# skywoodsz/qm_control

Measured on NVIDIA H100. Metric: mpc_wbc_iters_per_s, higher is better.
Workload: dtype f64

## Files before the change

### qm_control_b200/csrc/kernels/wbc_kernel.cu

```cuda
#include "dev_common.cuh"
#include "payload.cuh"
#include "wlinalg.cuh"

namespace qmb {

constexpr int LDM = 25;
constexpr int LDZ = 37;
constexpr int LZ = 19;
constexpr int MAXR = 24;
constexpr int LJC = 9;
constexpr int MAXW = 20;
#ifndef QMB_WBC_WARPS
#define QMB_WBC_WARPS 8
#endif
constexpr int WBC_WARPS = QMB_WBC_WARPS;

enum { ST_OK = 0, ST_ITER_CAP = 1, ST_TOO_MANY_ROWS = 2, ST_NAN = 4 };

struct EeWs { double Jee[6 * LDM], djv_ee[6], ee_m_pos[3], ee_m_vel[3], ee_m_rot[9], ee_m_w[3], ee_d_pos[3], ee_d_vel[3], ee_d_rot[9]; };
struct QpWs {
  union ZA { struct Q { double Z[36 * LZ];
                        double AR[MAXR * LDZ];
                      } q;
             RbdWs rbd;
             __device__ ZA() {} } za;
  union AH { double Ah[MAXR * LZ];
             EeWs ee; __device__ AH() {} } ah;
  double G[18 * 19 / 2 + 1];
  double tau[MAXR], tauc[MAXW];
  double xbar[36], dx[36], g[36], y[36], s[36], zac[LZ + 1], rhs[MAXR], bp[MAXR], bh[MAXR], lam[MAXW], t18[MAXR];
  int perm[MAXR], permc[MAXW], wset[MAXW];
};
static_assert(LZ * MAXR + LZ * MAXW <= MAXR * LDZ, "W1 and Wc share the row build area");
static_assert(sizeof(RbdWs) <= sizeof(double) * (36 * LZ + MAXR * LDZ), "rigid-body workspace overlays Z + AR only");

struct WbcSmem {
  double q[NQ], v[NQ], qd[NQ], vd[NQ];
  double M[NQ * LDM], nle[NQ];
  double Jc[12 * LJC], djv_f[12], fpos_m[12], fvel_m[12], fpos_d[12], fvel_d[12];
  double Tm[9], wdot_base[3], base_acc[6], fdes[12], lim[NJ], vstar[56];
  QpWs qp;
  Tuning tun;
};

struct IneqCtx { const WbcSmem* sm; int mode; int nc; double mu; int lfp, ffp; };
__device__ __forceinline__ int foot_first(int ffp, int f) { return (ffp >> (4 * f)) & 15; }
__device__ __forceinline__ double jt_force(const WbcSmem* sm, int lfp, int jn, const double* F) {
  if (jn >= 12) return 0.0;
  const int lg = jn / 3, f = (lfp >> (2 * lg)) & 3, d = jn - 3 * lg; const double* J = sm->Jc + 3 * f * LJC + 6 + d;
  return J[0] * F[3 * f] + J[LJC] * F[3 * f + 1] + J[2 * LJC] * F[3 * f + 2];
}

__device__ __forceinline__ int stance_foot_by_rank(int mode, int rank) { int k = 0; for (int f = 0; f < 4; ++f) if (contact_flag(mode, f)) { if (k == rank) return f; ++k; } return -1; }

__device__ __forceinline__ double ineq_row_dot(const IneqCtx& c, int i, const double* x) {
  if (i < 36) {
    const int jn = i < 18 ? i : i - 18; const double* Mr = c.sm->M + (6 + jn) * LDM; double s = 0.0;
    for (int k = 0; k < NQ; ++k) s += Mr[k] * x[k];
    s -= jt_force(c.sm, c.lfp, jn, x + NQ);
    return i < 18 ? s : -s;
  }
  const int r = i - 36; const int foot = stance_foot_by_rank(c.mode, r / 5); const int t = r % 5; const double* F = x + NQ + 3 * foot;
  if (t == 0) return -F[2];
  if (t == 1) return F[0] - c.mu * F[2];
  if (t == 2) return -F[0] - c.mu * F[2];
  if (t == 3) return F[1] - c.mu * F[2];
  return -F[1] - c.mu * F[2];
}
__device__ __forceinline__ double ineq_rhs(const IneqCtx& c, int i) {
  double f = 0.0;
  if (i < 18) f = c.sm->lim[i] - c.sm->nle[6 + i]; else if (i < 36) f = c.sm->lim[i - 18] + c.sm->nle[6 + i - 18];
  return f + c.sm->vstar[i];
}
__device__ __forceinline__ double ineq_row_elem(const IneqCtx& c, int i, int k) {
  if (i < 36) { const int jn = i < 18 ? i : i - 18; const double sgn = i < 18 ? 1.0 : -1.0; if (k < NQ) return sgn * c.sm->M[(6 + jn) * LDM + k];
    const int r = k - NQ, d = jn - foot_first(c.ffp, r / 3); return (d >= 0 && d < 3) ? -sgn * c.sm->Jc[r * LJC + 6 + d] : 0.0; }
  const int r = i - 36; const int foot = stance_foot_by_rank(c.mode, r / 5); const int t = r % 5; const int kk = k - NQ - 3 * foot;
  if (kk < 0 || kk > 2) return 0.0;
  if (kk == 2) return t == 0 ? -1.0 : -c.mu;
  if (kk == 0) return t == 1 ? 1.0 : (t == 2 ? -1.0 : 0.0);
  return t == 3 ? 1.0 : (t == 4 ? -1.0 : 0.0);
}

__device__ int cod_lstsq(QpWs& qp, double* W, int n, int r, int ldw, const double* rhs, double* y, double* G, int lane) {
  const int k = w_qrcp(W, n, r, ldw, qp.tau, qp.perm, 1e-11, lane);
  for (int i = lane; i < n; i += 32) y[i] = 0.0;
  __syncwarp();
  if (k == 0) return 0;
  if (k == r) {
    for (int c = 0; c < k; ++c) {
      double part = 0.0; if (lane < c) part = W[lane + c * ldw] * y[lane];
      const double s = warp_sum(part);
      if (lane == 0) y[c] = (rhs[qp.perm[c]] - s) / W[c + c * ldw];
      __syncwarp();
    }
  } else {
    { int a = 0, b = lane; while (b > a) { b -= a + 1; ++a; }
      while (a < k) { double s = 0.0; for (int c = a; c < r; ++c) s += W[a + c * ldw] * W[b + c * ldw]; G[tri(a) + b] = s;
        b += 32; while (b > a) { b -= a + 1; ++a; } } }
    if (lane < k) { double s = 0.0; for (int c = lane; c < r; ++c) s += W[lane + c * ldw] * rhs[qp.perm[c]]; qp.t18[lane] = s; }
    __syncwarp();
    w_cholesky(G, k, lane);
    w_chol_solve(G, k, qp.t18, lane);
    if (lane < k) y[lane] = qp.t18[lane];
    __syncwarp();
  }
  w_apply_q(W, n, k, ldw, qp.tau, y, lane);
  return k;
}

__device__ int build_level(WbcSmem& sm, const Tuning* __restrict__ tn, int level, int mode, int variant, bool init_phase, int ffp, int lane) {
  QpWs& qp = sm.qp; double* Ap = qp.za.q.AR; const EeWs& ee = qp.ah.ee; int nc = 0; for (int f = 0; f < 4; ++f) nc += contact_flag(mode, f);
  int rows = 0;
  if (level == 0) rows = 18;
  else if (level == 1) rows = (variant == 0) ? (init_phase ? 6 : 10 + 3 * (4 - nc)) : (6 + 3 * (4 - nc));
  else rows = (variant == 0) ? 14 : 12;
  for (int e = lane; e < rows * LDZ; e += 32) Ap[e] = 0.0;
  __syncwarp();
  if (level == 0) {
    for (int e = lane; e < 6 * 36; e += 32) { const int r = e / 36, k = e % 36; Ap[r * LDZ + k] = (k < NQ) ? sm.M[r * LDM + k] : -sm.Jc[(k - NQ) * LJC + r]; }
    if (lane < 6) qp.bp[lane] = -sm.nle[lane];
    int row = 6;
    for (int f = 0; f < 4; ++f) if (contact_flag(mode, f)) { if (lane < 27) { const int a = lane / 9, c = lane - 9 * a; Ap[(row + a) * LDZ + (c < 6 ? c : foot_first(ffp, f) + c)] = sm.Jc[(3 * f + a) * LJC + c]; } if (lane < 3) qp.bp[row + lane] = -sm.djv_f[3 * f + lane]; row += 3; }
    for (int f = 0; f < 4; ++f) if (!contact_flag(mode, f)) { if (lane < 3) { Ap[(row + lane) * LDZ + NQ + 3 * f + lane] = 1.0; qp.bp[row + lane] = 0.0; } row += 3; }
  } else if (level == 1) {
    int row = 0;
    if (variant == 0 && init_phase) {
      if (lane < 6) { const int k = NQ - 6 + lane; Ap[lane * LDZ + k] = 1.0; qp.bp[lane] = tn->arm_joint_kp[lane] * (sm.qd[k] - sm.q[k]) + tn->arm_joint_kd[lane] * (sm.vd[k] - sm.v[k]); }
      row = 6;
    } else {
      if (lane == 0) { Ap[2] = 1.0; qp.bp[0] = sm.base_acc[2] + tn->base_height_kp * (sm.qd[2] - sm.q[2]) + tn->base_height_kd * (sm.vd[2] - sm.v[2]); }
      if (lane < 3) {
        const int r = lane; for (int k = 0; k < 3; ++k) Ap[(1 + r) * LDZ + 3 + k] = sm.Tm[3 * r + k];
        double wM[3], wD[3]; matvec3(sm.Tm, sm.v + 3, wM); matvec3(sm.Tm, sm.vd + 3, wD);
        double Rm[9], Rr[9], err[3]; rot_zyx(sm.q[3], sm.q[4], sm.q[5], Rm); rot_zyx(sm.qd[3], sm.qd[4], sm.qd[5], Rr); rotation_error_world(Rr, Rm, err);
        double tdd[3], tde[3]; matvec3(sm.Tm, sm.base_acc + 3, tdd); euler_rate_map_dot_times(sm.q[3], sm.q[4], sm.vd + 3, tde);
        qp.bp[1 + r] = tdd[r] + tde[r] + tn->base_angular_kp * err[r] + tn->base_angular_kd * (wD[r] - wM[r]) - sm.wdot_base[r];
      }
      row = 4;
      if (variant == 0) {
        for (int e = lane; e < 6 * NQ; e += 32) { const int a = e / NQ, k = e % NQ; const bool zero = (a >= 3 && k >= 3 && k < 6); Ap[(row + a) * LDZ + k] = zero ? 0.0 : ee.Jee[a * LDM + k]; }
        if (lane < 3) qp.bp[row + lane] = tn->ee_linear_kp[lane] * (ee.ee_d_pos[lane] - ee.ee_m_pos[lane]) + tn->ee_linear_kd[lane] * (ee.ee_d_vel[lane] - ee.ee_m_vel[lane]) - ee.djv_ee[lane];
        if (lane == 3) { double err[3]; rotation_error_world(ee.ee_d_rot, ee.ee_m_rot, err);
          for (int a = 0; a < 3; ++a) qp.bp[row + 3 + a] = tn->ee_angular_kp[a] * err[a] - tn->ee_angular_kd[a] * ee.ee_m_w[a] - (ee.djv_ee[3 + a] - sm.wdot_base[a]); }
        row += 6;
      } else {
        if (lane < 2) { Ap[(row + lane) * LDZ + lane] = 1.0; qp.bp[row + lane] = sm.base_acc[lane] + tn->base_linear_kp * (sm.qd[lane] - sm.q[lane]) + tn->base_linear_kd * (sm.vd[lane] - sm.v[lane]); }
        row += 2;
      }
      for (int f = 0; f < 4; ++f) if (!contact_flag(mode, f)) {
        if (lane < 27) { const int a = lane / 9, c = lane - 9 * a; Ap[(row + a) * LDZ + (c < 6 ? c : foot_first(ffp, f) + c)] = 100.0 * sm.Jc[(3 * f + a) * LJC + c]; }
        if (lane < 3) { const int i = 3 * f + lane; qp.bp[row + lane] = 100.0 * (tn->kp_swing * (sm.fpos_d[i] - sm.fpos_m[i]) + tn->kd_swing * (sm.fvel_d[i] - sm.fvel_m[i]) - sm.djv_f[i]); }
        row += 3;
      }
    }
  } else {
    if (lane < 12) { Ap[lane * LDZ + NQ + lane] = 1.0; qp.bp[lane] = sm.fdes[lane]; }
    if (variant == 0 && lane < 2) { Ap[(12 + lane) * LDZ + lane] = 1.0; qp.bp[12 + lane] = sm.base_acc[lane] + tn->base_linear_kp * (sm.qd[lane] - sm.q[lane]) + tn->base_linear_kd * (sm.vd[lane] - sm.v[lane]); }
  }
  __syncwarp();
  return rows;
}

__device__ __forceinline__ void project_task(QpWs& qp, int rows, int off, int nz, int lane) {
  const double* Ap = qp.za.q.AR; const double* Z = qp.za.q.Z;
  for (int e = lane; e < rows * nz; e += 32) { const int i = e / nz, c = e - i * nz; const double* a = Ap + i * LDZ; double s0 = 0.0, s1 = 0.0;
#pragma unroll 6
    for (int k = 0; k < 36; k += 2) { s0 = fma(a[k], Z[k * LZ + off + c], s0); s1 = fma(a[k + 1], Z[(k + 1) * LZ + off + c], s1); }
    qp.ah.Ah[i * LZ + c] = s0 + s1; }
  if (lane < rows) { const double* a = Ap + lane * LDZ; double s = 0.0; for (int k = 0; k < 36; ++k) s = fma(a[k], qp.xbar[k], s); qp.bh[lane] = qp.bp[lane] - s; }
  __syncwarp();
}

__device__ int solve_level(WbcSmem& sm, const IneqCtx& ic, int rows, int off, int nzc, int& nw, int lane, int& iters_out, int iter_cap) {
  QpWs& qp = sm.qp; const int nz = nzc - off; const int nineq = 36 + 5 * ic.nc; int status = 0;
  if (nz <= 0) return 0;
  const double* Z = qp.za.q.Z; const double* Ah = qp.ah.Ah; double* W1 = qp.za.q.AR; double* Wc = qp.za.q.AR + LZ * MAXR;
  if (lane < LZ + 1) qp.zac[lane] = 0.0;
  __syncwarp();
  bool converged = false;
  for (int iter = 0; iter < iter_cap; ++iter) {
    iters_out = iter + 1;
    int kc = 0;
    if (nw > 0) {
      for (int k = 0; k < nw; ++k) {
        const int wi = qp.wset[k]; qp.y[lane] = ineq_row_elem(ic, wi, lane); if (lane < 4) qp.y[32 + lane] = ineq_row_elem(ic, wi, 32 + lane);
        __syncwarp();
        if (lane < nz) { double s0 = 0.0, s1 = 0.0;
#pragma unroll 6
          for (int j = 0; j < 36; j += 2) { s0 = fma(qp.y[j], Z[j * LZ + off + lane], s0); s1 = fma(qp.y[j + 1], Z[(j + 1) * LZ + off + lane], s1); }
          Wc[lane + k * LZ] = s0 + s1; }
        __syncwarp();
      }
      kc = w_qrcp(Wc, nz, nw, LZ, qp.tauc, qp.permc, 1e-10, lane);
      if (kc < nw) {
        int keep = (lane < kc) ? qp.wset[qp.permc[lane]] : -1; __syncwarp(); if (lane < kc) qp.wset[lane] = keep; nw = kc; __syncwarp();
        continue;
      }
    }
    for (int e = lane; e < rows * LZ; e += 32) W1[e] = Ah[e];
    if (lane < rows) { const double* a = Ah + lane * LZ; double s = 0.0; for (int c = 0; c < nz; ++c) s = fma(a[c], qp.zac[c], s); qp.rhs[lane] = qp.bh[lane] - s; }
    __syncwarp();
    if (kc > 0) w_apply_qt_cols(Wc, nz, kc, LZ, qp.tauc, W1, rows, LZ, lane);
    const int nfree = nz - kc;
    for (int i = lane; i < nz; i += 32) qp.s[i] = 0.0;
    __syncwarp();
    if (nfree > 0) cod_lstsq(qp, W1 + kc, nfree, rows, LZ, qp.rhs, qp.s + kc, qp.G, lane);
    if (kc > 0) w_apply_q(Wc, nz, kc, LZ, qp.tauc, qp.s, lane);
    for (int i = lane; i < 36; i += 32) { double d = 0.0; for (int c = 0; c < nz; ++c) d = fma(Z[i * LZ + off + c], qp.s[c], d); qp.dx[i] = d; }
    __syncwarp();
    double dmax = 0.0, xmax = 0.0; for (int i = lane; i < 36; i += 32) { dmax = fmax(dmax, fabs(qp.dx[i])); xmax = fmax(xmax, fabs(qp.xbar[i])); }
    dmax = warp_max(dmax); xmax = warp_max(xmax);
    bool full_step = true;
    if (dmax > 1e-12 * (1.0 + xmax)) {
      double alpha = 1.0; int blk = -1;
      for (int i = lane; i < nineq; i += 32) {
        bool inw = false; for (int k = 0; k < nw; ++k) inw |= (qp.wset[k] == i);
        if (inw) continue;
        const double ad = ineq_row_dot(ic, i, qp.dx);
        if (ad > 1e-12 * (1.0 + dmax)) { double r = (ineq_rhs(ic, i) - ineq_row_dot(ic, i, qp.xbar)) / ad; if (r < 0.0) r = 0.0; if (r < alpha) { alpha = r; blk = i; } }
      }
      { double a = alpha; int b = (blk < 0) ? 0x7fffffff : blk; warp_argmin(a, b); alpha = a; blk = (alpha < 1.0) ? b : -1; }
      for (int i = lane; i < 36; i += 32) qp.xbar[i] += alpha * qp.dx[i];
      if (lane < nz) qp.zac[lane] += alpha * qp.s[lane];
      __syncwarp();
      if (blk >= 0) { if (nw >= MAXW) { status |= ST_TOO_MANY_ROWS; break; } if (lane == 0) qp.wset[nw] = blk; nw += 1; __syncwarp(); full_step = false; }
    }
    if (!full_step) continue;
    if (nw == 0) { converged = true; break; }
    if (lane < rows) { const double* a = Ah + lane * LZ; double s = 0.0; for (int c = 0; c < nz; ++c) s = fma(a[c], qp.zac[c], s); qp.rhs[lane] = s - qp.bh[lane]; }
    __syncwarp();
    for (int c = lane; c < nz; c += 32) { double s = 0.0; for (int r = 0; r < rows; ++r) s = fma(Ah[r * LZ + c], qp.rhs[r], s); qp.g[c] = s; }
    __syncwarp();
    w_apply_qt(Wc, nz, kc, LZ, qp.tauc, qp.g, lane);
    double gmax = 0.0; for (int i = lane; i < nz; i += 32) gmax = fmax(gmax, fabs(qp.g[i])); gmax = warp_max(gmax);
    for (int c = kc - 1; c >= 0; --c) {
      double part = 0.0; if (lane > c && lane < kc) part = Wc[c + lane * LZ] * qp.lam[lane];
      const double s = warp_sum(part);
      if (lane == 0) qp.lam[c] = (-qp.g[c] - s) / Wc[c + c * LZ];
      __syncwarp();
    }
    double lmin = (lane < kc) ? qp.lam[lane] : 1e300; int li = lane; warp_argmin(lmin, li);
    if (lmin >= -1e-9 * (1.0 + gmax)) { converged = true; break; }
    { const int drop = qp.permc[li]; int keep = -1; if (lane < nw) { int src = lane < drop ? lane : lane + 1; keep = (src < nw) ? qp.wset[src] : -1; } __syncwarp(); if (lane < nw - 1) qp.wset[lane] = keep;
      nw -= 1; __syncwarp(); }
  }
  if (!converged) status |= ST_ITER_CAP;
  return status;
}

template <bool TUNED>
__global__ void __launch_bounds__(32 * WBC_WARPS) wbc_update_kernel(const DevModel* __restrict__ mdl, int b0, int B, const double* __restrict__ x_des, const double* __restrict__ u_des,
                                                                   const double* __restrict__ rbd_meas, const int32_t* __restrict__ mode_in, const double* __restrict__ period_in,
                                                                   const double* __restrict__ time_in, double* __restrict__ input_last, int variant,
                                                                   double* __restrict__ cmd_out, int32_t* __restrict__ status_out, int32_t* __restrict__ diag_out,
                                                                   const double* __restrict__ srbd, const double* __restrict__ payload, const double* __restrict__ tuning) {
  extern __shared__ __align__(16) unsigned char smem_raw[];
  const int warp = threadIdx.x >> 5, lane = threadIdx.x & 31;
  const int b = b0 + blockIdx.x * (int)(blockDim.x >> 5) + warp;
  if (b >= B) return;
  WbcSmem& sm = reinterpret_cast<WbcSmem*>(smem_raw)[warp];
  const int mode = mode_in[b]; const double period = period_in[b]; const double time = time_in[b];
  int nc = 0; for (int f = 0; f < 4; ++f) nc += contact_flag(mode, f);

  const double* xdes = x_des + (size_t)b * NX; const double* udes = u_des + (size_t)b * NU;
  if (lane < 12) sm.fdes[lane] = udes[lane];
  const int lfp = mdl->leg_foot[0] | (mdl->leg_foot[1] << 2) | (mdl->leg_foot[2] << 4) | (mdl->leg_foot[3] << 6);
  const int ffp = mdl->foot_leg[0] | (mdl->foot_leg[1] << 4) | (mdl->foot_leg[2] << 8) | (mdl->foot_leg[3] << 12);
  if (lane < NJ) sm.lim[lane] = (lane < 12) ? mdl->effort[lane % 3] : mdl->effort[lane];
  for (int i = lane; i < 56; i += 32) sm.vstar[i] = 0.0;
  rbd_read(rbd_meas + (size_t)b * 55, sm.q, sm.v, sm.Tm, lane);
  if (lane < NQ) sm.qd[lane] = xdes[6 + lane];
  __syncwarp();

  RbdWs* ws = &sm.qp.za.rbd; EeWs& ee = sm.qp.ah.ee;
  rbd_kinematics<true>(mdl, sm.q, sm.v, ws, lane);
  rbd_inertias(mdl, ws, lane, 1);
  if (payload) { if (lane < 2) payload_load(mdl, ws, lane, payload + (size_t)b * 8 + 4 * lane, true); __syncwarp(); }
  rbd_accumulate(mdl, ws, lane, true);
  rbd_mass_matrix_nle(mdl, ws, sm.M, LDM, sm.nle, lane);
  for (int f = 0; f < 4; ++f) {
    const int body = mdl->foot_body[f]; double pw[3]; foot_point(mdl, ws, f, pw);
    if (lane < 9) { const double* S = ws->S[lane < 6 ? lane : foot_first(ffp, f) + lane]; double col[3]; point_vel(S, pw, col);
      for (int a = 0; a < 3; ++a) sm.Jc[(3 * f + a) * LJC + lane] = col[a]; }
    if (lane == 0) { double vel[3], acc[3]; point_vel_acc(ws->V[body], ws->A[body], pw, vel, acc); for (int a = 0; a < 3; ++a) { sm.fpos_m[3 * f + a] = pw[a]; sm.fvel_m[3 * f + a] = vel[a]; sm.djv_f[3 * f + a] = acc[a]; } }
  }
  {
    const int body = mdl->ee_body; double pw[3]; ee_pose(mdl, ws, pw, lane == 0 ? ee.ee_m_rot : nullptr);
    point_jacobian(ws, pw, 12, 17, ee.Jee, LDM, lane);
    if (lane < NQ) { const bool on = (lane < 6) || (lane >= 18); for (int a = 0; a < 3; ++a) ee.Jee[(3 + a) * LDM + lane] = on ? ws->S[lane][a] : 0.0; }
    if (lane == 0) { double vel[3], acc[3]; point_vel_acc(ws->V[body], ws->A[body], pw, vel, acc); for (int a = 0; a < 3; ++a) { ee.ee_m_pos[a] = pw[a]; ee.ee_m_vel[a] = vel[a]; ee.djv_ee[a] = acc[a]; ee.djv_ee[3 + a] = ws->A[body][a]; ee.ee_m_w[a] = ws->V[body][a]; sm.wdot_base[a] = ws->A[0][a]; } }
  }
  __syncwarp();

  double jacc = 0.0;
  if (lane < NJ) { const double uj = udes[12 + lane]; jacc = (uj - input_last[(size_t)b * NU + 12 + lane]) / period; sm.vd[6 + lane] = uj; }
  __syncwarp();
  if (lane < NU) input_last[(size_t)b * NU + lane] = udes[lane];
  double A22inv[9], A12[9];
  if (lane == 0) {
    const SrbdConst* sc = srbd_of(mdl, srbd, b);
    double R[9], T[9]; rot_zyx(sm.qd[3], sm.qd[4], sm.qd[5], R); euler_rate_map(sm.qd[3], sm.qd[4], T);
    double c[3]; matvec3(R, sc->c_nom, c);
    double RI[9], RIRt[9], A22[9]; matmul3(R, sc->I_nom, RI); matmul3_nt(RI, R, RIRt); matmul3(RIRt, T, A22); inv3(A22, A22inv);
    const double Sx[9] = {0, -c[2], c[1], c[2], 0, -c[0], -c[1], c[0], 0}; double ST[9]; matmul3(Sx, T, ST); for (int i = 0; i < 9; ++i) A12[i] = sc->m * ST[i];
    double ha[3] = {sc->m * xdes[3], sc->m * xdes[4], sc->m * xdes[5]}, ed[3]; matvec3(A22inv, ha, ed);
    double t[3]; matvec3(A12, ed, t);
    for (int a = 0; a < 3; ++a) { sm.vd[a] = xdes[a] - t[a] / sc->m; sm.vd[3 + a] = ed[a]; }
  }
  __syncwarp();
  rbd_kinematics<true>(mdl, sm.qd, sm.vd, ws, lane);
  rbd_inertias(mdl, ws, lane, 2);
  if (payload) { if (lane < 2) payload_load(mdl, ws, lane, payload + (size_t)b * 8 + 4 * lane, false); __syncwarp(); }
  rbd_accumulate(mdl, ws, lane, true);
  double Phi[6] = {0, 0, 0, 0, 0, 0};
  if (lane < NJ) { inertia_apply(ws->Ic[lane + 1], ws->S[6 + lane], Phi); for (int i = 0; i < 6; ++i) Phi[i] *= jacc; }
  for (int i = 0; i < 6; ++i) Phi[i] = warp_sum(Phi[i]);
  for (int f = 0; f < 4; ++f) {
    double pw[3]; foot_point(mdl, ws, f, pw);
    if (lane == 0) { double vel[3]; point_vel(ws->V[mdl->foot_body[f]], pw, vel); for (int a = 0; a < 3; ++a) { sm.fpos_d[3 * f + a] = pw[a]; sm.fvel_d[3 * f + a] = vel[a]; } }
  }
  if (lane == 0) {
    double pw[3], vel[3]; ee_pose(mdl, ws, pw, ee.ee_d_rot); point_vel(ws->V[mdl->ee_body], pw, vel);
    for (int a = 0; a < 3; ++a) { ee.ee_d_pos[a] = pw[a]; ee.ee_d_vel[a] = vel[a]; }
    const SrbdConst* sc = srbd_of(mdl, srbd, b);
    const double mt = ws->Ic[0][0]; const double com[3] = {ws->Ic[0][1] / mt, ws->Ic[0][2] / mt, ws->Ic[0][3] / mt};
    double lin[3] = {0, 0, -9.81 * sc->m}, ang[3] = {0, 0, 0};
    for (int f = 0; f < 4; ++f) { const double* F = sm.fdes + 3 * f; const double r[3] = {sm.fpos_d[3 * f] - com[0], sm.fpos_d[3 * f + 1] - com[1], sm.fpos_d[3 * f + 2] - com[2]}; lin[0] += F[0]; lin[1] += F[1]; lin[2] += F[2]; cross3_add(r, F, ang); }
    const double* Fb = ws->F[0]; double cf[3]; cross3(com, Fb + 3, cf);
    double cp[3]; cross3(com, Phi + 3, cp);
    for (int a = 0; a < 3; ++a) { lin[a] -= Fb[3 + a] + Phi[3 + a]; ang[a] -= (Fb[a] - cf[a]) + (Phi[a] - cp[a]); }
    double ed[3]; matvec3(A22inv, ang, ed); double t[3]; matvec3(A12, ed, t);
    for (int a = 0; a < 3; ++a) { sm.base_acc[a] = (lin[a] - t[a]) / sc->m; sm.base_acc[3 + a] = ed[a]; }
  }
  __syncwarp();

  if (TUNED) { const double* tr = tuning + (size_t)b * TUNING_DBL; for (int i = lane; i < TUNING_MODEL; i += 32) reinterpret_cast<double*>(&sm.tun)[i] = tr[i]; }
  const Tuning* tn = TUNED ? &sm.tun : tuning_of(mdl, nullptr, 0);
  QpWs& qp = sm.qp; IneqCtx ic{&sm, mode, nc, TUNED ? tuning[(size_t)b * TUNING_DBL + 1] : mdl->wbc_friction, lfp, ffp}; int status = 0;
  const bool init_phase = time < 10.0;
  double* AR = qp.za.q.AR; double* Z = qp.za.q.Z;
  for (int i = lane; i < 36; i += 32) qp.xbar[i] = 0.0;
  __syncwarp();
  const int nineq = 36 + 5 * nc; const int cap0 = mdl->wbc_iter_cap0, cap = mdl->wbc_iter_cap; int it0 = 0;
  unsigned vmask0 = 0, vmask1 = 0;
  int k0 = 0;
  for (int it = 0; it < cap0; ++it) {
    int r = build_level(sm, tn, 0, mode, variant, init_phase, ffp, lane); it0 = it + 1;
    for (int i = 0; i < nineq; ++i) { const bool in = (i < 32) ? ((vmask0 >> i) & 1u) : ((vmask1 >> (i - 32)) & 1u); if (in) { if (r >= MAXR) { status |= ST_TOO_MANY_ROWS; break; }
        for (int k = lane; k < 36; k += 32) AR[r * LDZ + k] = ineq_row_elem(ic, i, k); if (lane == 0) qp.bp[r] = ineq_rhs(ic, i); ++r; } }
    __syncwarp();
    k0 = cod_lstsq(qp, AR, 36, r, LDZ, qp.bp, qp.xbar, Z, lane);
    __syncwarp();
    unsigned n0 = 0, n1 = 0;
    for (int i = lane; i < nineq; i += 32) { const double val = ineq_row_dot(ic, i, qp.xbar) - ineq_rhs(ic, i); const double sc = 1e-9 * (1.0 + fabs(ineq_rhs(ic, i)));
      const bool inV = (i < 32) ? ((vmask0 >> i) & 1u) : ((vmask1 >> (i - 32)) & 1u);
      if (val > sc || (inV && val >= -sc)) { if (i < 32) n0 |= 1u << i; else n1 |= 1u << (i - 32); } }
    for (int o = 16; o > 0; o >>= 1) { n0 |= __shfl_xor_sync(FULL, n0, o); n1 |= __shfl_xor_sync(FULL, n1, o); }
    if (n0 == vmask0 && n1 == vmask1) break;
    vmask0 = n0; vmask1 = n1;
    if (it == cap0 - 1) status |= ST_ITER_CAP;
  }
  for (int i = lane; i < nineq; i += 32) { const double val = ineq_row_dot(ic, i, qp.xbar) - ineq_rhs(ic, i); sm.vstar[i] = val > 0.0 ? val : 0.0; }
  __syncwarp();
  int off = 0, nzc = 0, nw = 0, it1 = 0, it2 = 0;
  {
    if (vmask0 | vmask1) {
      const int rows0 = build_level(sm, tn, 0, mode, variant, init_phase, ffp, lane);
      k0 = w_qrcp(AR, 36, rows0, LDZ, qp.tau, qp.perm, 1e-11, lane);
    }
    nzc = 36 - k0;
    if (nzc > LZ - 1) { status |= ST_TOO_MANY_ROWS; nzc = 0; }
    else w_form_q_tail(AR, 36, k0, LDZ, qp.tau, Z, LZ, lane);
  }
  for (int level = 1; level <= 2 && nzc > 0; ++level) {
    const int rows = build_level(sm, tn, level, mode, variant, init_phase, ffp, lane);
    const int nz = nzc - off;
    if (nz <= 0) break;
    project_task(qp, rows, off, nz, lane);
    status |= solve_level(sm, ic, rows, off, nzc, nw, lane, level == 1 ? it1 : it2, cap);
    if (level == 1) {
      const int k = w_qrcp(qp.ah.Ah, nz, rows, LZ, qp.tau, qp.perm, 1e-11, lane);
      w_apply_q_right(qp.ah.Ah, nz, k, LZ, qp.tau, Z, 36, LZ, off, lane);
      off += k;
    }
  }
  double* out = cmd_out + (size_t)b * 54;
  for (int i = lane; i < 36; i += 32) out[i] = qp.xbar[i];
  bool bad = false;
  if (lane < NJ) { const double* Mr = sm.M + (6 + lane) * LDM; double s = sm.nle[6 + lane]; for (int k = 0; k < NQ; ++k) s += Mr[k] * qp.xbar[k]; s -= jt_force(&sm, lfp, lane, qp.xbar + NQ); out[36 + lane] = s; bad = !isfinite(s); }
  if (__any_sync(FULL, bad)) status |= ST_NAN;
  if (lane == 0) { status_out[b] = status; if (diag_out) diag_out[b] = (it0 & 0xff) | ((it1 & 0xff) << 8) | ((it2 & 0xff) << 16) | ((nw & 0xff) << 24); }
}

static_assert(sizeof(WbcSmem) * WBC_WARPS <= 227 * 1024, "WBC shared-memory budget exceeded");
size_t wbc_smem_bytes() { return sizeof(WbcSmem) * WBC_WARPS; }

void launch_wbc_update(const DevModel* mdl, int B, const double* x_des, const double* u_des, const double* rbd, const int32_t* mode, const double* period, const double* time,
                       double* input_last, int variant, double* cmd, int32_t* status, cudaStream_t stream, int b0, int b1, int32_t* diag, const double* srbd, const double* payload, const double* tuning) {
  if (b1 < 0) b1 = B; if (b1 <= b0) return;
  const int nb = b1 - b0; const int wpc = WBC_WARPS;
  const int grid = (nb + wpc - 1) / wpc;
  (tuning ? wbc_update_kernel<true> : wbc_update_kernel<false>)<<<grid, 32 * wpc, sizeof(WbcSmem) * wpc, stream>>>(mdl, b0, b1, x_des, u_des, rbd, mode, period, time, input_last, variant, cmd, status, diag, srbd, payload, tuning);
}

int wbc_configure_device() {
  cudaError_t e = cudaFuncSetAttribute(wbc_update_kernel<false>, cudaFuncAttributeMaxDynamicSharedMemorySize, (int)wbc_smem_bytes());
  if (e == cudaSuccess) e = cudaFuncSetAttribute(wbc_update_kernel<true>, cudaFuncAttributeMaxDynamicSharedMemorySize, (int)wbc_smem_bytes());
  return (int)e;
}

}
```

### qm_control_b200/csrc/kernels/wlinalg.cuh

```cuda
#pragma once
#include "dev_common.cuh"

#ifndef QMB_QRCP_NORMS
#define QMB_QRCP_NORMS 2
#endif

namespace qmb {


__device__ __forceinline__ int w_qrcp(double* W, int n, int r, int ld, double* tau, int* perm, double tol_rel, int lane) {
  if (lane < r) perm[lane] = lane;
  double vn = 0.0;
  if (lane < r) for (int i = 0; i < n; ++i) { const double x = W[i + lane * ld]; vn += x * x; }
  double vref = vn;
  const double thresh = tol_rel * tol_rel * warp_max(vn);
  const int kmax = n < r ? n : r; int rank = kmax;
  __syncwarp();
  for (int j = 0; j < kmax; ++j) {
#if QMB_QRCP_NORMS == 0
    if (lane >= j && lane < r) { vn = 0.0; for (int i = j; i < n; ++i) { const double x = W[i + lane * ld]; vn += x * x; } }
#endif
    double nr = vn; int pc = lane;
    warp_argmax_nonneg(nr, pc, lane >= j && lane < r);
    if (!(nr > thresh)) { rank = j; break; }
    if (pc != j) {
      for (int i = lane; i < n; i += 32) { const double t = W[i + j * ld]; W[i + j * ld] = W[i + pc * ld]; W[i + pc * ld] = t; }
      if (lane == 0) { const int t = perm[j]; perm[j] = perm[pc]; perm[pc] = t; }
      const double vj = __shfl_sync(FULL, vn, j), rj = __shfl_sync(FULL, vref, j);
      if (lane == pc) { vn = vj; vref = rj; }
    }
    __syncwarp();
#if QMB_QRCP_NORMS == 1
    {
      double part = 0.0; for (int i = j + lane; i < n; i += 32) { const double x = W[i + j * ld]; part += x * x; }
      nr = warp_sum(part);
      if (!(nr > thresh)) { rank = j; break; }
    }
#endif
    const double x0 = W[j + j * ld]; const double beta = (x0 >= 0.0) ? -sqrt(nr) : sqrt(nr);
    const double d = x0 - beta, inv = 1.0 / (beta * d);
    const double tj = -d * d * inv; const double scal = beta * inv;
    __syncwarp();
    for (int i = j + 1 + lane; i < n; i += 32) W[i + j * ld] *= scal;
    if (lane == 0) { W[j + j * ld] = beta; tau[j] = tj; }
    __syncwarp();
    if (lane > j && lane < r) {
      double* col = W + lane * ld; const double* v = W + j * ld;
      double w = col[j]; for (int i = j + 1; i < n; ++i) w += v[i] * col[i];
      w *= tj; const double cj = col[j] - w; col[j] = cj;
#if QMB_QRCP_NORMS == 2
      double nn = 0.0; for (int i = j + 1; i < n; ++i) { const double c = fma(-w, v[i], col[i]); col[i] = c; nn = fma(c, c, nn); }
      vn = nn;
#else
      for (int i = j + 1; i < n; ++i) col[i] -= w * v[i];
#endif
#if QMB_QRCP_NORMS == 1
      vn = fmax(vn - cj * cj, 0.0);
      if (vref > 0.0 && vn <= 1.4901161193847656e-8 * vref) {
        vn = 0.0; for (int i = j + 1; i < n; ++i) { const double x = col[i]; vn += x * x; }
        if (!(vn > thresh)) vn = 0.0;
        vref = vn;
      }
#endif
    }
    __syncwarp();
  }
  return rank;
}

__device__ __forceinline__ void w_apply_qt(const double* W, int n, int k, int ld, const double* tau, double* g, int lane) {
  for (int j = 0; j < k; ++j) {
    const double* v = W + j * ld; double part = 0.0;
    for (int i = j + lane; i < n; i += 32) part += (i == j ? 1.0 : v[i]) * g[i];
    const double w = tau[j] * warp_sum(part);
    for (int i = j + lane; i < n; i += 32) g[i] -= w * (i == j ? 1.0 : v[i]);
    __syncwarp();
  }
}
__device__ __forceinline__ void w_apply_q(const double* W, int n, int k, int ld, const double* tau, double* g, int lane) {
  for (int j = k - 1; j >= 0; --j) {
    const double* v = W + j * ld; double part = 0.0;
    for (int i = j + lane; i < n; i += 32) part += (i == j ? 1.0 : v[i]) * g[i];
    const double w = tau[j] * warp_sum(part);
    for (int i = j + lane; i < n; i += 32) g[i] -= w * (i == j ? 1.0 : v[i]);
    __syncwarp();
  }
}
__device__ __forceinline__ void w_apply_qt_cols(const double* W, int n, int k, int ld, const double* tau, double* C, int ncols, int ldc, int lane) {
  if (lane < ncols) {
    double* col = C + lane * ldc;
    for (int j = 0; j < k; ++j) {
      const double* v = W + j * ld; double w = col[j]; for (int i = j + 1; i < n; ++i) w = fma(v[i], col[i], w);
      w *= tau[j]; col[j] -= w; for (int i = j + 1; i < n; ++i) col[i] = fma(-w, v[i], col[i]);
    }
  }
  __syncwarp();
}
__device__ __forceinline__ void w_apply_q_right(const double* W, int n, int k, int ld, const double* tau, double* Z, int rows, int ldz, int off, int lane) {
  for (int j = 0; j < k; ++j) {
    const double* v = W + j * ld; const double tj = tau[j];
    for (int i = lane; i < rows; i += 32) {
      double* zr = Z + i * ldz + off; double d = zr[j]; for (int c = j + 1; c < n; ++c) d += zr[c] * v[c];
      d *= tj; zr[j] -= d; for (int c = j + 1; c < n; ++c) zr[c] -= d * v[c];
    }
    __syncwarp();
  }
}

__device__ __forceinline__ void w_form_q_tail(const double* W, int n, int k, int ld, const double* tau, double* Z, int ldz, int lane) {
  const int nc = n - k;
  if (lane < nc) {
    double* col = Z + lane;
    for (int i = 0; i < n; ++i) col[i * ldz] = (i == k + lane) ? 1.0 : 0.0;
    for (int j = k - 1; j >= 0; --j) {
      const double* v = W + j * ld; double w0 = col[j * ldz], w1 = 0.0; int i = j + 1;
      for (; i + 1 < n; i += 2) { w0 = fma(v[i], col[i * ldz], w0); w1 = fma(v[i + 1], col[(i + 1) * ldz], w1); }
      if (i < n) w0 = fma(v[i], col[i * ldz], w0);
      const double w = (w0 + w1) * tau[j]; col[j * ldz] -= w; for (int i2 = j + 1; i2 < n; ++i2) col[i2 * ldz] = fma(-w, v[i2], col[i2 * ldz]);
    }
  }
  __syncwarp();
}

__device__ __forceinline__ int tri(int a) { return (a * (a + 1)) >> 1; }
__device__ __forceinline__ bool w_cholesky(double* A, int n, int lane) {
  bool ok = true;
  for (int j = 0; j < n; ++j) {
    const double d = A[tri(j) + j];
    if (!(d > 0.0)) { ok = false; break; }
    const double s = sqrt(d);
    __syncwarp();
    double* row = A + tri(lane);
    if (lane == j) row[j] = s;
    if (lane > j && lane < n) row[j] /= s;
    __syncwarp();
    if (lane > j && lane < n) { const double lij = row[j]; int oc = tri(j + 1) + j; for (int c = j + 1; c <= lane; ++c) { row[c] -= lij * A[oc]; oc += c + 1; } }
    __syncwarp();
  }
  return ok;
}
__device__ __forceinline__ void w_chol_solve(const double* L, int n, double* b, int lane) {
  const double* row = L + tri(lane);
  for (int j = 0; j < n; ++j) {
    if (lane == j) b[j] /= row[j];
    __syncwarp();
    if (lane > j && lane < n) b[lane] -= row[j] * b[j];
    __syncwarp();
  }
  for (int j = n - 1; j >= 0; --j) {
    if (lane == j) b[j] /= row[j];
    __syncwarp();
    if (lane < j) b[lane] -= L[tri(j) + lane] * b[j];
    __syncwarp();
  }
}

}
```

Before: 24.37.

## Update working-set QR incrementally and reuse level-0 factorisation across passes

The active-set QP inner loop now keeps Ah and zac in the rotated basis and appends a newly blocking constraint to the existing Householder QR of the working set. Previously it re-projected every working constraint and reran a full pivoted QR on each iteration; a full refactorisation now happens only after a constraint is dropped or an append is rank-deficient. The level-0 factorisation from the first semismooth pass is cached in Z/bh and restored later instead of being rebuilt, and several dot-product loops are split into two or four accumulators. In exchange the numerics change slightly, there is extra rotate/unrotate bookkeeping, and the cached factorisation depends on aliasing shared workspace correctly.

```diff
diff --git a/qm_control_b200/csrc/kernels/wbc_kernel.cu b/qm_control_b200/csrc/kernels/wbc_kernel.cu
--- a/qm_control_b200/csrc/kernels/wbc_kernel.cu
+++ b/qm_control_b200/csrc/kernels/wbc_kernel.cu
@@ -32,6 +32,7 @@
   int perm[MAXR], permc[MAXW], wset[MAXW];
 };
 static_assert(LZ * MAXR + LZ * MAXW <= MAXR * LDZ, "W1 and Wc share the row build area");
+static_assert(18 * 36 <= 36 * LZ && 18 <= MAXR, "Z and bh hold the level-0 factorisation of A0 (18 rows) between the semismooth passes");
 static_assert(sizeof(RbdWs) <= sizeof(double) * (36 * LZ + MAXR * LDZ), "rigid-body workspace overlays Z + AR only");
 
 struct WbcSmem {
@@ -172,42 +173,68 @@
   __syncwarp();
 }
 
+__device__ __forceinline__ double project_ineq_row(QpWs& qp, const IneqCtx& ic, int i, int off, int nz, int lane) {
+  const double* Z = qp.za.q.Z;
+  qp.y[lane] = ineq_row_elem(ic, i, lane); if (lane < 4) qp.y[32 + lane] = ineq_row_elem(ic, i, 32 + lane);
+  __syncwarp();
+  double d = 0.0;
+  if (lane < nz) { double s0 = 0.0, s1 = 0.0, s2 = 0.0, s3 = 0.0;
+#pragma unroll 3
+    for (int j = 0; j < 36; j += 4) { s0 = fma(qp.y[j], Z[j * LZ + off + lane], s0); s1 = fma(qp.y[j + 1], Z[(j + 1) * LZ + off + lane], s1);
+                                      s2 = fma(qp.y[j + 2], Z[(j + 2) * LZ + off + lane], s2); s3 = fma(qp.y[j + 3], Z[(j + 3) * LZ + off + lane], s3); }
+    d = (s0 + s1) + (s2 + s3); }
+  __syncwarp();
+  return d;
+}
+
 __device__ int solve_level(WbcSmem& sm, const IneqCtx& ic, int rows, int off, int nzc, int& nw, int lane, int& iters_out, int iter_cap) {
   QpWs& qp = sm.qp; const int nz = nzc - off; const int nineq = 36 + 5 * ic.nc; int status = 0;
   if (nz <= 0) return 0;
-  const double* Z = qp.za.q.Z; const double* Ah = qp.ah.Ah; double* W1 = qp.za.q.AR; double* Wc = qp.za.q.AR + LZ * MAXR;
+  const double* Z = qp.za.q.Z; double* Ah = qp.ah.Ah; double* W1 = qp.za.q.AR; double* Wc = qp.za.q.AR + LZ * MAXR;
   if (lane < LZ + 1) qp.zac[lane] = 0.0;
   __syncwarp();
+  int kc = 0;
+  bool refactor = nw > 0;
+  double cmax = 0.0;
   bool converged = false;
   for (int iter = 0; iter < iter_cap; ++iter) {
     iters_out = iter + 1;
-    int kc = 0;
-    if (nw > 0) {
-      for (int k = 0; k < nw; ++k) {
-        const int wi = qp.wset[k]; qp.y[lane] = ineq_row_elem(ic, wi, lane); if (lane < 4) qp.y[32 + lane] = ineq_row_elem(ic, wi, 32 + lane);
-        __syncwarp();
-        if (lane < nz) { double s0 = 0.0, s1 = 0.0;
-#pragma unroll 6
-          for (int j = 0; j < 36; j += 2) { s0 = fma(qp.y[j], Z[j * LZ + off + lane], s0); s1 = fma(qp.y[j + 1], Z[(j + 1) * LZ + off + lane], s1); }
-          Wc[lane + k * LZ] = s0 + s1; }
-        __syncwarp();
-      }
+    if (!refactor && nw > kc) {
+      const double c = project_ineq_row(qp, ic, qp.wset[kc], off, nz, lane);
+      cmax = fmax(cmax, warp_sum(c * c));
+      if (w_qr_append(Wc, nz, kc, LZ, qp.tauc, c, 1e-20 * cmax, lane)) {
+        w_apply_qt_cols(Wc, nz, kc + 1, LZ, qp.tauc, Ah, rows, LZ, lane, kc); w_apply_qt(Wc, nz, kc + 1, LZ, qp.tauc, qp.zac, lane, kc);
+        kc += 1;
+      } else refactor = true;
+    }
+    if (refactor) {
+      refactor = false;
+      if (kc > 0) { w_apply_q_cols(Wc, nz, kc, LZ, qp.tauc, Ah, rows, LZ, lane); w_apply_q(Wc, nz, kc, LZ, qp.tauc, qp.zac, lane); }
+      for (int k = 0; k < nw; ++k) { const double c = project_ineq_row(qp, ic, qp.wset[k], off, nz, lane); if (lane < nz) Wc[lane + k * LZ] = c; }
+      __syncwarp();
       kc = w_qrcp(Wc, nz, nw, LZ, qp.tauc, qp.permc, 1e-10, lane);
-      if (kc < nw) {
-        int keep = (lane < kc) ? qp.wset[qp.permc[lane]] : -1; __syncwarp(); if (lane < kc) qp.wset[lane] = keep; nw = kc; __syncwarp();
-        continue;
-      }
+      { double n2 = 0.0; if (lane < kc) for (int i = 0; i <= lane; ++i) n2 = fma(Wc[i + lane * LZ], Wc[i + lane * LZ], n2); cmax = warp_max(n2); }
+      const bool dependent = kc < nw;
+      { int keep = (lane < kc) ? qp.wset[qp.permc[lane]] : -1; __syncwarp(); if (lane < kc) qp.wset[lane] = keep; nw = kc; __syncwarp(); }
+      if (kc > 0) { w_apply_qt_cols(Wc, nz, kc, LZ, qp.tauc, Ah, rows, LZ, lane); w_apply_qt(Wc, nz, kc, LZ, qp.tauc, qp.zac, lane); }
+      if (dependent) continue;
     }
     for (int e = lane; e < rows * LZ; e += 32) W1[e] = Ah[e];
-    if (lane < rows) { const double* a = Ah + lane * LZ; double s = 0.0; for (int c = 0; c < nz; ++c) s = fma(a[c], qp.zac[c], s); qp.rhs[lane] = qp.bh[lane] - s; }
-    __syncwarp();
-    if (kc > 0) w_apply_qt_cols(Wc, nz, kc, LZ, qp.tauc, W1, rows, LZ, lane);
+    if (lane < rows) { const double* a = Ah + lane * LZ; double s0 = 0.0, s1 = 0.0; int c = 0;
+      for (; c + 1 < nz; c += 2) { s0 = fma(a[c], qp.zac[c], s0); s1 = fma(a[c + 1], qp.zac[c + 1], s1); }
+      if (c < nz) s0 = fma(a[c], qp.zac[c], s0);
+      qp.rhs[lane] = qp.bh[lane] - (s0 + s1); }
     const int nfree = nz - kc;
     for (int i = lane; i < nz; i += 32) qp.s[i] = 0.0;
     __syncwarp();
     if (nfree > 0) cod_lstsq(qp, W1 + kc, nfree, rows, LZ, qp.rhs, qp.s + kc, qp.G, lane);
-    if (kc > 0) w_apply_q(Wc, nz, kc, LZ, qp.tauc, qp.s, lane);
-    for (int i = lane; i < 36; i += 32) { double d = 0.0; for (int c = 0; c < nz; ++c) d = fma(Z[i * LZ + off + c], qp.s[c], d); qp.dx[i] = d; }
+    for (int i = lane; i < nz; i += 32) qp.y[i] = qp.s[i];
+    __syncwarp();
+    if (kc > 0) w_apply_q(Wc, nz, kc, LZ, qp.tauc, qp.y, lane);
+    for (int i = lane; i < 36; i += 32) { double d0 = 0.0, d1 = 0.0; int c = 0;
+      for (; c + 1 < nz; c += 2) { d0 = fma(Z[i * LZ + off + c], qp.y[c], d0); d1 = fma(Z[i * LZ + off + c + 1], qp.y[c + 1], d1); }
+      if (c < nz) d0 = fma(Z[i * LZ + off + c], qp.y[c], d0);
+      qp.dx[i] = d0 + d1; }
     __syncwarp();
     double dmax = 0.0, xmax = 0.0; for (int i = lane; i < 36; i += 32) { dmax = fmax(dmax, fabs(qp.dx[i])); xmax = fmax(xmax, fabs(qp.xbar[i])); }
     dmax = warp_max(dmax); xmax = warp_max(xmax);
@@ -228,11 +255,16 @@
     }
     if (!full_step) continue;
     if (nw == 0) { converged = true; break; }
-    if (lane < rows) { const double* a = Ah + lane * LZ; double s = 0.0; for (int c = 0; c < nz; ++c) s = fma(a[c], qp.zac[c], s); qp.rhs[lane] = s - qp.bh[lane]; }
-    __syncwarp();
-    for (int c = lane; c < nz; c += 32) { double s = 0.0; for (int r = 0; r < rows; ++r) s = fma(Ah[r * LZ + c], qp.rhs[r], s); qp.g[c] = s; }
-    __syncwarp();
-    w_apply_qt(Wc, nz, kc, LZ, qp.tauc, qp.g, lane);
+    if (lane < rows) { const double* a = Ah + lane * LZ; double s0 = 0.0, s1 = 0.0; int c = 0;
+      for (; c + 1 < nz; c += 2) { s0 = fma(a[c], qp.zac[c], s0); s1 = fma(a[c + 1], qp.zac[c + 1], s1); }
+      if (c < nz) s0 = fma(a[c], qp.zac[c], s0);
+      qp.rhs[lane] = (s0 + s1) - qp.bh[lane]; }
+    __syncwarp();
+    for (int c = lane; c < nz; c += 32) { double s0 = 0.0, s1 = 0.0; int r = 0;
+      for (; r + 1 < rows; r += 2) { s0 = fma(Ah[r * LZ + c], qp.rhs[r], s0); s1 = fma(Ah[(r + 1) * LZ + c], qp.rhs[r + 1], s1); }
+      if (r < rows) s0 = fma(Ah[r * LZ + c], qp.rhs[r], s0);
+      qp.g[c] = s0 + s1; }
+    __syncwarp();
     double gmax = 0.0; for (int i = lane; i < nz; i += 32) gmax = fmax(gmax, fabs(qp.g[i])); gmax = warp_max(gmax);
     for (int c = kc - 1; c >= 0; --c) {
       double part = 0.0; if (lane > c && lane < kc) part = Wc[c + lane * LZ] * qp.lam[lane];
@@ -242,9 +274,11 @@
     }
     double lmin = (lane < kc) ? qp.lam[lane] : 1e300; int li = lane; warp_argmin(lmin, li);
     if (lmin >= -1e-9 * (1.0 + gmax)) { converged = true; break; }
-    { const int drop = qp.permc[li]; int keep = -1; if (lane < nw) { int src = lane < drop ? lane : lane + 1; keep = (src < nw) ? qp.wset[src] : -1; } __syncwarp(); if (lane < nw - 1) qp.wset[lane] = keep;
+    { int keep = -1; if (lane < nw) { int src = lane < li ? lane : lane + 1; keep = (src < nw) ? qp.wset[src] : -1; } __syncwarp(); if (lane < nw - 1) qp.wset[lane] = keep;
       nw -= 1; __syncwarp(); }
-  }
+    refactor = true;
+  }
+  if (kc > 0) w_apply_q_cols(Wc, nz, kc, LZ, qp.tauc, Ah, rows, LZ, lane);
   if (!converged) status |= ST_ITER_CAP;
   return status;
 }
@@ -345,6 +379,7 @@
   const int nineq = 36 + 5 * nc; const int cap0 = mdl->wbc_iter_cap0, cap = mdl->wbc_iter_cap; int it0 = 0;
   unsigned vmask0 = 0, vmask1 = 0;
   int k0 = 0;
+  int k00 = -1, r00 = 0;
   for (int it = 0; it < cap0; ++it) {
     int r = build_level(sm, tn, 0, mode, variant, init_phase, ffp, lane); it0 = it + 1;
     for (int i = 0; i < nineq; ++i) { const bool in = (i < 32) ? ((vmask0 >> i) & 1u) : ((vmask1 >> (i - 32)) & 1u); if (in) { if (r >= MAXR) { status |= ST_TOO_MANY_ROWS; break; }
@@ -352,12 +387,18 @@
     __syncwarp();
     k0 = cod_lstsq(qp, AR, 36, r, LDZ, qp.bp, qp.xbar, Z, lane);
     __syncwarp();
+    if (it > 0 && k0 > 0 && k0 < r) k00 = -1;
     unsigned n0 = 0, n1 = 0;
     for (int i = lane; i < nineq; i += 32) { const double val = ineq_row_dot(ic, i, qp.xbar) - ineq_rhs(ic, i); const double sc = 1e-9 * (1.0 + fabs(ineq_rhs(ic, i)));
       const bool inV = (i < 32) ? ((vmask0 >> i) & 1u) : ((vmask1 >> (i - 32)) & 1u);
       if (val > sc || (inV && val >= -sc)) { if (i < 32) n0 |= 1u << i; else n1 |= 1u << (i - 32); } }
     for (int o = 16; o > 0; o >>= 1) { n0 |= __shfl_xor_sync(FULL, n0, o); n1 |= __shfl_xor_sync(FULL, n1, o); }
     if (n0 == vmask0 && n1 == vmask1) break;
+    if (it == 0) {
+      for (int e = lane; e < r * 36; e += 32) { const int c = e / 36, i = e - 36 * c; Z[e] = AR[c * LDZ + i]; }
+      if (lane < r) qp.bh[lane] = qp.tau[lane];
+      k00 = k0; r00 = r; __syncwarp();
+    }
     vmask0 = n0; vmask1 = n1;
     if (it == cap0 - 1) status |= ST_ITER_CAP;
   }
@@ -366,8 +407,14 @@
   int off = 0, nzc = 0, nw = 0, it1 = 0, it2 = 0;
   {
     if (vmask0 | vmask1) {
-      const int rows0 = build_level(sm, tn, 0, mode, variant, init_phase, ffp, lane);
-      k0 = w_qrcp(AR, 36, rows0, LDZ, qp.tau, qp.perm, 1e-11, lane);
+      if (k00 >= 0) {
+        for (int e = lane; e < r00 * 36; e += 32) { const int c = e / 36, i = e - 36 * c; AR[c * LDZ + i] = Z[e]; }
+        if (lane < r00) qp.tau[lane] = qp.bh[lane];
+        k0 = k00; __syncwarp();
+      } else {
+        const int rows0 = build_level(sm, tn, 0, mode, variant, init_phase, ffp, lane);
+        k0 = w_qrcp(AR, 36, rows0, LDZ, qp.tau, qp.perm, 1e-11, lane);
+      }
     }
     nzc = 36 - k0;
     if (nzc > LZ - 1) { status |= ST_TOO_MANY_ROWS; nzc = 0; }
diff --git a/qm_control_b200/csrc/kernels/wlinalg.cuh b/qm_control_b200/csrc/kernels/wlinalg.cuh
--- a/qm_control_b200/csrc/kernels/wlinalg.cuh
+++ b/qm_control_b200/csrc/kernels/wlinalg.cuh
@@ -11,7 +11,10 @@
 __device__ __forceinline__ int w_qrcp(double* W, int n, int r, int ld, double* tau, int* perm, double tol_rel, int lane) {
   if (lane < r) perm[lane] = lane;
   double vn = 0.0;
-  if (lane < r) for (int i = 0; i < n; ++i) { const double x = W[i + lane * ld]; vn += x * x; }
+  if (lane < r) { double v0 = 0.0, v1 = 0.0; int i = 0;
+    for (; i + 1 < n; i += 2) { const double x0 = W[i + lane * ld], x1 = W[i + 1 + lane * ld]; v0 = fma(x0, x0, v0); v1 = fma(x1, x1, v1); }
+    if (i < n) { const double x = W[i + lane * ld]; v0 = fma(x, x, v0); }
+    vn = v0 + v1; }
   double vref = vn;
   const double thresh = tol_rel * tol_rel * warp_max(vn);
   const int kmax = n < r ? n : r; int rank = kmax;
@@ -46,11 +49,16 @@
     __syncwarp();
     if (lane > j && lane < r) {
       double* col = W + lane * ld; const double* v = W + j * ld;
-      double w = col[j]; for (int i = j + 1; i < n; ++i) w += v[i] * col[i];
+      double w0 = col[j], w1 = 0.0; int i = j + 1;
+      for (; i + 1 < n; i += 2) { w0 = fma(v[i], col[i], w0); w1 = fma(v[i + 1], col[i + 1], w1); }
+      if (i < n) w0 = fma(v[i], col[i], w0);
+      double w = w0 + w1;
       w *= tj; const double cj = col[j] - w; col[j] = cj;
 #if QMB_QRCP_NORMS == 2
-      double nn = 0.0; for (int i = j + 1; i < n; ++i) { const double c = fma(-w, v[i], col[i]); col[i] = c; nn = fma(c, c, nn); }
-      vn = nn;
+      double n0 = 0.0, n1 = 0.0; i = j + 1;
+      for (; i + 1 < n; i += 2) { const double c0 = fma(-w, v[i], col[i]), c1 = fma(-w, v[i + 1], col[i + 1]); col[i] = c0; col[i + 1] = c1; n0 = fma(c0, c0, n0); n1 = fma(c1, c1, n1); }
+      if (i < n) { const double c = fma(-w, v[i], col[i]); col[i] = c; n0 = fma(c, c, n0); }
+      vn = n0 + n1;
 #else
       for (int i = j + 1; i < n; ++i) col[i] -= w * v[i];
 #endif
@@ -68,8 +76,8 @@
   return rank;
 }
 
-__device__ __forceinline__ void w_apply_qt(const double* W, int n, int k, int ld, const double* tau, double* g, int lane) {
-  for (int j = 0; j < k; ++j) {
+__device__ __forceinline__ void w_apply_qt(const double* W, int n, int k, int ld, const double* tau, double* g, int lane, int j0 = 0) {
+  for (int j = j0; j < k; ++j) {
     const double* v = W + j * ld; double part = 0.0;
     for (int i = j + lane; i < n; i += 32) part += (i == j ? 1.0 : v[i]) * g[i];
     const double w = tau[j] * warp_sum(part);
@@ -86,16 +94,42 @@
     __syncwarp();
   }
 }
-__device__ __forceinline__ void w_apply_qt_cols(const double* W, int n, int k, int ld, const double* tau, double* C, int ncols, int ldc, int lane) {
+__device__ __forceinline__ void w_apply_qt_cols(const double* W, int n, int k, int ld, const double* tau, double* C, int ncols, int ldc, int lane, int j0 = 0) {
   if (lane < ncols) {
     double* col = C + lane * ldc;
-    for (int j = 0; j < k; ++j) {
+    for (int j = j0; j < k; ++j) {
       const double* v = W + j * ld; double w = col[j]; for (int i = j + 1; i < n; ++i) w = fma(v[i], col[i], w);
       w *= tau[j]; col[j] -= w; for (int i = j + 1; i < n; ++i) col[i] = fma(-w, v[i], col[i]);
     }
   }
   __syncwarp();
 }
+__device__ __forceinline__ void w_apply_q_cols(const double* W, int n, int k, int ld, const double* tau, double* C, int ncols, int ldc, int lane) {
+  if (lane < ncols) {
+    double* col = C + lane * ldc;
+    for (int j = k - 1; j >= 0; --j) {
+      const double* v = W + j * ld; double w = col[j]; for (int i = j + 1; i < n; ++i) w = fma(v[i], col[i], w);
+      w *= tau[j]; col[j] -= w; for (int i = j + 1; i < n; ++i) col[i] = fma(-w, v[i], col[i]);
+    }
+  }
+  __syncwarp();
+}
+__device__ __forceinline__ bool w_qr_append(double* W, int n, int k, int ld, double* tau, double c, double thresh, int lane) {
+  for (int j = 0; j < k; ++j) {
+    const double v = (lane == j) ? 1.0 : ((lane > j && lane < n) ? W[lane + j * ld] : 0.0);
+    const double w = tau[j] * warp_sum(v * c);
+    c = fma(-w, v, c);
+  }
+  const double nr = warp_sum((lane >= k && lane < n) ? c * c : 0.0);
+  if (!(nr > thresh)) return false;
+  const double x0 = __shfl_sync(FULL, c, k); const double beta = (x0 >= 0.0) ? -sqrt(nr) : sqrt(nr);
+  const double d = x0 - beta, inv = 1.0 / (beta * d);
+  if (lane == k) { c = beta; tau[k] = -d * d * inv; } else if (lane > k) c *= beta * inv;
+  if (lane < n) W[lane + k * ld] = c;
+  __syncwarp();
+  return true;
+}
+
 __device__ __forceinline__ void w_apply_q_right(const double* W, int n, int k, int ld, const double* tau, double* Z, int rows, int ldz, int off, int lane) {
   for (int j = 0; j < k; ++j) {
     const double* v = W + j * ld; const double tj = tau[j];
```

New measurement: 24.64, median of 6. 1.1% higher.
